# shahruk10/kaldi-tflite

Measured on AMD Instinct MI355X. Metric: x-vectors/sec (10 s @16 kHz), higher is better.
Workload: dtype f16mx

## Files before the change

### kaldi-tflite_amd/csrc/tdnn_mx.hip

```cpp
#include "tdnn_mx_common.h"

#define MXP_ROWS 256
__global__ __launch_bounds__(MXP_ROWS) void mx_planes_kernel(const float* __restrict__ src, int64_t T, int64_t ld, int D,
                                                             const int32_t* __restrict__ lens, char* __restrict__ xh,
                                                             char* __restrict__ xl4, char* __restrict__ x4, char* __restrict__ xs) {
    __shared__ float tile[MXP_ROWS * 33];
    const int b = blockIdx.z, c = blockIdx.y, nch = gridDim.y;
    const int64_t t0 = (int64_t)blockIdx.x * MXP_ROWS;
    const int64_t len = lens ? (int64_t)lens[b] : T;
    if (t0 >= len) return;
    const int rows = (int)(len - t0 < MXP_ROWS ? len - t0 : MXP_ROWS);
    const int tid = threadIdx.x;
    const float* base = src + ((int64_t)b * T + t0) * ld + c * 32;
    const bool vec = (ld & 3) == 0 && ((uintptr_t)src & 15) == 0 && c * 32 + 32 <= ld;
#pragma unroll
    for (int k = 0; k < 8; ++k) {
        const int q = k * MXP_ROWS + tid, r = q >> 3, e4 = (q & 7) * 4;
        if (r < rows) {
            float v[4];
            if (vec) {
                const f32x4 t = *reinterpret_cast<const f32x4*>(base + (int64_t)r * ld + e4);
                const int nd = D - (c * 32 + e4);
                v[0] = nd > 0 ? t.x : 0.0f; v[1] = nd > 1 ? t.y : 0.0f; v[2] = nd > 2 ? t.z : 0.0f; v[3] = nd > 3 ? t.w : 0.0f;
            } else {
#pragma unroll
                for (int e = 0; e < 4; ++e) v[e] = (c * 32 + e4 + e < D) ? base[(int64_t)r * ld + e4 + e] : 0.0f;
            }
#pragma unroll
            for (int e = 0; e < 4; ++e) tile[r * 33 + e4 + e] = __builtin_amdgcn_fmed3f(v[e], -65504.0f, 65504.0f);
        }
    }
    __syncthreads();
    const int64_t rec0 = ((int64_t)b * nch + c) * T + t0;
    u32x4 hp[4];
    if (tid < rows) {
        float v[32];
#pragma unroll
        for (int e = 0; e < 32; ++e) v[e] = tile[tid * 33 + e];
        u32x4 l4, h4;
        unsigned sw;
        mx_encode32(v, hp, l4, h4, sw);
        *reinterpret_cast<u32x4*>(xl4 + (rec0 + tid) * 16) = l4;
        *reinterpret_cast<u32x4*>(x4 + (rec0 + tid) * 16) = h4;
        *reinterpret_cast<unsigned*>(xs + (rec0 + tid) * 4) = sw;
    }
    __syncthreads();
    unsigned* himg = reinterpret_cast<unsigned*>(tile);
    if (tid < rows) {
#pragma unroll
        for (int k = 0; k < 4; ++k) *reinterpret_cast<u32x4*>(himg + tid * 20 + k * 4) = hp[k];
    }
    __syncthreads();
#pragma unroll
    for (int k = 0; k < 4; ++k) {
        const int q = k * MXP_ROWS + tid, r = q >> 2;
        if (r < rows)
            *reinterpret_cast<u32x4*>(xh + rec0 * 64 + (int64_t)q * 16) = *reinterpret_cast<const u32x4*>(himg + r * 20 + (q & 3) * 4);
    }
}

extern "C" int ktf_mx_planes(const float* src, int64_t B, int64_t T, int32_t D, int64_t ld_src, const int32_t* lens, void* xh,
                             void* xl4, void* x4, void* xs, void* stream) {
    KTF_REQUIRE(B >= 0 && T >= 0 && D > 0 && ld_src >= D, "ktf_mx_planes: bad size");
    if (B == 0 || T == 0) return KTF_OK;
    KTF_REQUIRE(src && xh && xl4 && x4 && xs, "ktf_mx_planes: null argument");
    const int nch = (D + 31) / 32;
    KTF_REQUIRE(B < 65536 && nch < 65536, "ktf_mx_planes: B and D / 32 must be below 65536");
    hipLaunchKernelGGL(mx_planes_kernel, dim3((unsigned)((T + MXP_ROWS - 1) / MXP_ROWS), (unsigned)nch, (unsigned)B), dim3(MXP_ROWS), 0,
                       (hipStream_t)stream, src, T, ld_src, (int)D, lens, (char*)xh, (char*)xl4, (char*)x4, (char*)xs);
    KTF_CHECK_LAUNCH("ktf_mx_planes");
    return KTF_OK;
}

template <int ACT, int OUT, bool PADK, bool FLAT = false>
__device__ __forceinline__ void mx_tile(const MxParams& p, const int id, int mtiles, int ntiles, int gtiles, double* __restrict__ stats,
                                        unsigned char* rsm) {
    static_assert(!FLAT || OUT != MX_OUT_F32, "flat row tiles: plane output or fused pooling");
#define MX_ARG_BATCH()                                                                                                                     \
    asm volatile("" ::"s"(p.xh), "s"(p.wh), "s"(p.T), "s"(p.nss), "s"(p.nk), "s"(p.nctx), "s"(p.nch_in), "s"(p.ctx_pk[0]), "s"(p.ctx_pk[1]), \
                 "s"(p.t_div_m), "s"(p.t_div_s), "s"(p.start), "s"(p.sub), "s"(p.cut))
    const int xcd = id & 7, slot = id >> 3;
    const int g = (slot / ntiles) * 8 + xcd;
    const int nt = slot - (slot / ntiles) * ntiles;
    if (g >= gtiles) return;
    const int b = FLAT ? 0 : g / mtiles, mt = FLAT ? g : g - b * mtiles;
    const int n0 = nt * 256, t0 = FLAT ? 0 : mt * 256;
    const int tid = threadIdx.x, lane = tid & 63;
    const int wave = __builtin_amdgcn_readfirstlane(tid >> 6);
    const int wm = wave >> 2, wn = wave & 3;
    const int R0 = mt * 256;
    int len, out_len;
    [[maybe_unused]] bool dense = false;
    if constexpr (FLAT) {
        const int total = p.row_starts[mtiles];
        MX_ARG_BATCH();
        if (R0 >= total) return;
        len = (int)p.T;
        out_len = total - R0 < 256 ? total - R0 : 256;
        dense = total == mtiles * len;
    } else {
        len = p.lens ? p.lens[b] : (int)p.T;
        MX_ARG_BATCH();
        out_len = len - p.cut - p.start <= 0 ? 0 : (len - p.cut - p.start + p.sub - 1) / p.sub;
        if (t0 >= out_len) return;
    }
    const int lenm1 = len - 1;
    const int64_t ub = FLAT ? 0 : (int64_t)b * p.nch_in * p.T;
    const int nkp = p.nss * 4;
    const __amdgpu_buffer_rsrc_t r_xh = mx_rsrc_pinned(p.xh + (ub - MX_KQ_BIAS) * 64);
    const __amdgpu_buffer_rsrc_t r_wh = mx_rsrc_pinned(p.wh + (int64_t)nt * nkp * MX_TILE);
    const __amdgpu_buffer_rsrc_t r_wq = mx_rsrc_pinned(p.wq + (int64_t)nt * p.nss * MX_WQ_BLOCK);

    unsigned a_cb[2];
    int a_row[2];
#pragma unroll
    for (int i = 0; i < 2; ++i) {
        const int q = i * 512 + tid;
        const int row = q >> 2;
        a_cb[i] = (unsigned)(((q & 3) ^ ((4 - ((row >> 2) & 3)) & 3)) * 16);
        a_row[i] = p.start + (t0 + row) * p.sub;
    }
    [[maybe_unused]] int a_lm1[2] = {lenm1, lenm1}, s_lm1 = lenm1;
    int s_row = p.start + (t0 + lane + 64 * (wave & 3)) * p.sub;
    [[maybe_unused]] unsigned a_ub[2] = {0u, 0u}, s_ub = 0u;
    [[maybe_unused]] auto flat_row = [&](int m) -> i32x4 {
        if (dense) {
            const int R = R0 + m;
            if (m >= out_len) return i32x4{-1, 0, 1, 0};
            const int bb = p.t_div_m ? (int)(__umulhi((unsigned)R, p.t_div_m) >> p.t_div_s) : R;
            return i32x4{R, R - bb * len, len, bb};
        }
        return reinterpret_cast<const i32x4*>(p.row_map)[R0 + m];
    };
    const unsigned long long cpk0 = p.ctx_pk[0], cpk1 = p.ctx_pk[1];
#define MX_CTX(ci_) ((int)(signed char)(((ci_) < 8 ? cpk0 : cpk1) >> (((ci_) & 7) * 8)))
    [[maybe_unused]] bool interior = false;
    if constexpr (FLAT) {
        i32x4 er[3];
        const int mr[3] = {tid >> 2, (512 + tid) >> 2, lane + 64 * (wave & 3)};
        if (dense) {
#pragma unroll
            for (int i = 0; i < 3; ++i) er[i] = flat_row(mr[i]);
        } else {
#pragma unroll
            for (int i = 0; i < 3; ++i) er[i] = reinterpret_cast<const i32x4*>(p.row_map)[R0 + mr[i]];
        }
#pragma unroll
        for (int i = 0; i < 2; ++i) {
            a_row[i] = er[i].y;
            a_lm1[i] = er[i].z - 1;
            a_ub[i] = er[i].x < 0 ? 0u : (unsigned)(er[i].x - er[i].y) * (unsigned)p.nch_in;
        }
        s_row = er[2].y;
        s_lm1 = er[2].z - 1;
        s_ub = er[2].x < 0 ? 0u : (unsigned)(er[2].x - er[2].y) * (unsigned)p.nch_in;
    }
    const unsigned vw = (unsigned)tid * 16u;
    const int wave_k0 = (int)(unsigned)(size_t)(lds_ptr_t*)(rsm + wave * 1024);
    [[maybe_unused]] const int wave_k = wave_k0;
#define MX_LDS_AT(off_, c_) ((lds_ptr_t*)(size_t)(unsigned)((off_) + (c_)))
    int kb[5], ko[5];
    kb[0] = MX_KQ_BIAS;
    ko[0] = MX_CTX(0);
#define MX_DMA_A_E(ks_, e_, n_)                                                                                        \
    {                                                                                                                  \
        int r_ = a_row[n_] + ko[e_];                                                                                   \
        const int hi_ = FLAT ? a_lm1[n_] : lenm1;                                                                      \
        r_ = r_ < 0 ? 0 : (r_ > hi_ ? hi_ : r_);                                                                       \
        const unsigned vo_ = ((FLAT ? a_ub[n_] : 0u) + (unsigned)r_) * 64u + a_cb[n_];                                 \
        __builtin_amdgcn_raw_ptr_buffer_load_lds(r_xh, MX_LDS_AT(wave_k, ((ks_) & 1) * MX_STAGE + (n_) * 8192), 16, vo_, kb[e_] << 6, 0, 0); \
    }
#define MX_DMA_A_I(ks_, e_, n_)                                                                                        \
    __builtin_amdgcn_raw_ptr_buffer_load_lds(r_xh, MX_LDS_AT(wave_k, ((ks_) & 1) * MX_STAGE + (n_) * 8192), 16, (n_) ? va1 : va0, \
                                             (kb[e_] + ko[e_]) << 6, 0, 0);
#define MX_DMA_A(ks_, e_, n_) { if constexpr (INTERIOR) MX_DMA_A_I(ks_, e_, n_) else MX_DMA_A_E(ks_, e_, n_) }
#define MX_DMA_W(ks_, n_)                                                                                              \
    __builtin_amdgcn_raw_ptr_buffer_load_lds(r_wh, MX_LDS_AT(wave_k, ((ks_) & 1) * MX_STAGE + MX_TILE + (n_) * 8192), 16, vw, \
                                             (ks_) * MX_TILE + (n_) * 8192, 0, 0);
    MX_DMA_W(0, 0) MX_DMA_W(0, 1) MX_DMA_A_E(0, 0, 0) MX_DMA_A_E(0, 0, 1)
    const __amdgpu_buffer_rsrc_t r_xl4 = mx_rsrc_pinned(p.xl4 + (ub - MX_KQ_BIAS) * 16);
    const __amdgpu_buffer_rsrc_t r_x4 = mx_rsrc_pinned(p.x4 + (ub - MX_KQ_BIAS) * 16);
    const __amdgpu_buffer_rsrc_t r_xs = mx_rsrc_pinned(p.xs + (ub - MX_KQ_BIAS) * 4);
    if constexpr (FLAT) {
        if (p.nctx == 1 && MX_CTX(0) == 0) {
            interior = true;
        } else if (out_len == 256) {
            const i32x4 e0 = flat_row(0), e1 = flat_row(255);
            interior = __builtin_amdgcn_readfirstlane(e0.w) == __builtin_amdgcn_readfirstlane(e1.w) &&
                       __builtin_amdgcn_readfirstlane(e0.y) + MX_CTX(0) >= 0 &&
                       __builtin_amdgcn_readfirstlane(e1.y) + MX_CTX(p.nctx - 1) <= __builtin_amdgcn_readfirstlane(e1.z) - 1;
        }
    }
    [[maybe_unused]] const unsigned va0 = (a_ub[0] + (unsigned)a_row[0]) * 64u + a_cb[0], va1 = (a_ub[1] + (unsigned)a_row[1]) * 64u + a_cb[1];
    [[maybe_unused]] const unsigned vs16 = (s_ub + (unsigned)s_row) * 16u, vs4 = (s_ub + (unsigned)s_row) * 4u;

    const int sa_k0 = (int)(unsigned)(size_t)(lds_ptr_t*)(rsm + (wave & 3) * 1024 + (wave >> 2) * 4096);
    const int sa_ks0 = (int)(unsigned)(size_t)(lds_ptr_t*)(rsm + (wave & 3) * 256 + (wave >> 2) * 1024);
    const bool wave_hi = wave >= 4;

    int* const tkb = reinterpret_cast<int*>(rsm + MX_KQ_OFF);
    int* const tko = tkb + (nkp + 4);

#define MX_DMA_SA(n_)                                                                                                  \
    {                                                                                                                  \
        constexpr int plane_ = ((n_) < 4 ? (n_) : 0) >> 1, h_ = (n_) < 4 ? ((n_) & 1) : (n_) - 4;                      \
        unsigned rec_ = 0u;                                                                                            \
        int so_;                                                                                                       \
        if constexpr (INTERIOR) {                                                                                      \
            so_ = sk_b[h_] + sk_o[h_];                                                                                 \
        } else {                                                                                                       \
            int r_ = s_row + sk_o[h_];                                                                                 \
            const int hi_ = FLAT ? s_lm1 : lenm1;                                                                      \
            r_ = r_ < 0 ? 0 : (r_ > hi_ ? hi_ : r_);                                                                   \
            rec_ = (FLAT ? s_ub : 0u) + (unsigned)r_;                                                                  \
            so_ = sk_b[h_];                                                                                            \
        }                                                                                                              \
        if ((n_) < 4) {                                                                                                \
            __builtin_amdgcn_raw_ptr_buffer_load_lds(plane_ ? r_x4 : r_xl4, MX_LDS_AT(sa_k, MX_SA_OFF + plane_ * 16384 + h_ * 8192), 16, \
                                                     INTERIOR ? vs16 : rec_ * 16u, so_ << 4, 0, 0);                    \
        } else {                                                                                                       \
            __builtin_amdgcn_raw_ptr_buffer_load_lds(r_xs, MX_LDS_AT(sa_ks, MX_SA_OFF + 32768 + h_ * 2048), 4, INTERIOR ? vs4 : rec_ * 4u, so_ << 2, 0, 0); \
        }                                                                                                              \
    }
#define MX_DMA_SW(ss_, n_)                                                                                             \
    __builtin_amdgcn_raw_ptr_buffer_load_lds(r_wq, MX_LDS_AT(wave_k, MX_SW_OFF + (n_) * 8192), 16, vw, (ss_) * MX_WQ_BLOCK + (n_) * 8192, 0, 0);

    f32x4 acc[8][4];
    const int r16 = lane & 15, q4 = lane >> 4;
    const int fr = (4 - ((r16 >> 2) & 3)) & 3;
    const int coff = ((q4 ^ fr) << 4);
    const int a_row_off = (wm * 128 + r16) * 64 + coff;
    const int b_row_off = (wn * 64 + r16) * 64 + coff;
    const int klim = PADK ? p.nk : nkp;

    auto kloop = [&](auto itag) {
        constexpr bool INTERIOR = decltype(itag)::value;
        {
            unsigned char* const prm_w = rsm + MX_PRM_OFF + (wave & 3) * 256;
            const unsigned vcol = (unsigned)(n0 + (wave & 3) * 64 + lane) * 4u;
            const float* const vec0 = wave_hi ? p.scale : p.bias;
            if (vec0) __builtin_amdgcn_raw_ptr_buffer_load_lds(mx_rsrc(vec0, p.units * 4), (lds_ptr_t*)(prm_w + (wave_hi ? 1024 : 0)), 4, vcol, 0, 0, 0);
            else reinterpret_cast<float*>(prm_w + (wave_hi ? 1024 : 0))[lane] = wave_hi ? 1.0f : 0.0f;
            if (!wave_hi) {
                if (p.shift) __builtin_amdgcn_raw_ptr_buffer_load_lds(mx_rsrc(p.shift, p.units * 4), (lds_ptr_t*)(prm_w + 2048), 4, vcol, 0, 0, 0);
                else reinterpret_cast<float*>(prm_w + 2048)[lane] = 0.0f;
            }
        }
        for (int k = tid; k < nkp + 4; k += 512) {
            const int kk = k + 1 < p.nk ? k + 1 : 0;
            const int ch = kk / p.nctx, ci = kk - ch * p.nctx;
            tkb[k] = ch * (int)p.T + MX_KQ_BIAS;
            tko[k] = MX_CTX(ci);
        }
        {
            int ch = 0, ci = 0;
#pragma unroll
            for (int e = 1; e <= 4; ++e) {
                if (++ci == p.nctx) { ci = 0; ++ch; }
                const bool real = e < p.nk;
                kb[e] = (real ? ch * (int)p.T : 0) + MX_KQ_BIAS;
                ko[e] = real ? MX_CTX(ci) : MX_CTX(0);
            }
        }
#pragma unroll
        for (int i = 0; i < 8; ++i)
#pragma unroll
            for (int j = 0; j < 4; ++j) acc[i][j] = f32x4{0.0f, 0.0f, 0.0f, 0.0f};
        for (int ss = 0; ss < p.nss; ++ss) {
            i32x4 tb_n, to_n;
            int sk_b[2], sk_o[2];
            int wave_k = wave_k0, sa_k = sa_k0, sa_ks = sa_ks0;
            asm volatile("" : "+s"(wave_k), "+s"(sa_k), "+s"(sa_ks));
#pragma unroll
            for (int j = 0; j < 4; ++j) {
                const int ks = 4 * ss + j;
                if (j == 1 || j == 2) asm volatile("s_waitcnt vmcnt(6)" ::: "memory");
                else if (j == 0) asm volatile("s_waitcnt vmcnt(0) lgkmcnt(0)" ::: "memory");
                else asm volatile("s_waitcnt vmcnt(0)" ::: "memory");
                __builtin_amdgcn_s_barrier();
                asm volatile("" ::: "memory");
                const bool live = PADK ? ks < p.nk : true;
#define MX_NEXT() ({ int k1_ = ks + 1; asm volatile("" : "+s"(k1_)); k1_ < klim; })
                const unsigned char* sa = rsm + (ks & 1) * MX_STAGE;
                const unsigned char* sw = sa + MX_TILE;
                hfrag8 bh[4];
                hfrag8 a_cur, a_nx1;
                if (live) {
#pragma unroll
                    for (int jj = 0; jj < 4; ++jj) bh[jj] = *reinterpret_cast<const hfrag8*>(sw + b_row_off + jj * 1024);
                    a_cur = *reinterpret_cast<const hfrag8*>(sa + a_row_off);
                    a_nx1 = *reinterpret_cast<const hfrag8*>(sa + a_row_off + 1024);
                }
                __builtin_amdgcn_sched_barrier(0);
                if (MX_NEXT()) { MX_DMA_A(ks + 1, j + 1, 0) MX_DMA_A(ks + 1, j + 1, 1) }
                __builtin_amdgcn_sched_barrier(0);
#pragma unroll
                for (int i = 0; i < 8; ++i) {
                    if (live) {
                        acc[i][0] = __builtin_amdgcn_mfma_f32_16x16x32_f16(a_cur, bh[0], acc[i][0], 0, 0, 0);
                        __builtin_amdgcn_sched_barrier(0);
                        hfrag8 a_nx2 = a_nx1;
                        if (i < 6) a_nx2 = *reinterpret_cast<const hfrag8*>(sa + a_row_off + (i + 2) * 1024);
#pragma unroll
                        for (int jj = 1; jj < 4; ++jj) acc[i][jj] = __builtin_amdgcn_mfma_f32_16x16x32_f16(a_cur, bh[jj], acc[i][jj], 0, 0, 0);
                        a_cur = a_nx1;
                        a_nx1 = a_nx2;
                    }
                    __builtin_amdgcn_sched_barrier(0);
                    if (i == 0) { if (MX_NEXT()) MX_DMA_W(ks + 1, 0) }
                    if (i == 1) { if (MX_NEXT()) MX_DMA_W(ks + 1, 1) }
                    if (j == 0) {
                        if (i == 1) {
                            sk_b[0] = wave_hi ? kb[1] : kb[0]; sk_o[0] = wave_hi ? ko[1] : ko[0];
                            sk_b[1] = wave_hi ? kb[3] : kb[2]; sk_o[1] = wave_hi ? ko[3] : ko[2];
                        }
                        if (i == 2) MX_DMA_SA(0)
                        if (i == 3) MX_DMA_SA(1)
                        if (i == 4) MX_DMA_SA(2)
                        if (i == 5) MX_DMA_SA(3)
                        if (i == 6) MX_DMA_SA(4)
                        if (i == 7) MX_DMA_SA(5)
                    }
                    if (j == 1) {
                        if (i == 2) MX_DMA_SW(ss, 0)
                        if (i == 3) MX_DMA_SW(ss, 1)
                        if (i == 4) MX_DMA_SW(ss, 2)
                        if (i == 5) MX_DMA_SW(ss, 3)
                        if (i == 6) MX_DMA_SW(ss, 4)
                        if (i == 7) MX_DMA_SW(ss, 5)
                    }
                    if (j == 2 && i == 3) {
                        tb_n = *reinterpret_cast<const i32x4*>(tkb + 4 * ss + 4);
                        to_n = *reinterpret_cast<const i32x4*>(tko + 4 * ss + 4);
                    }
                    __builtin_amdgcn_sched_barrier(0);
                }
#undef MX_NEXT
            }
            __builtin_amdgcn_sched_barrier(0);
            {
                int tl;
                asm volatile("v_mbcnt_lo_u32_b32 %0, -1, 0\n\tv_mbcnt_hi_u32_b32 %0, -1, %0" : "=v"(tl));
                const int sw_rec = ((tl & 63) >> 4) * 256 + wn * 64 + (tl & 15);
                const int sa_rec = ((tl & 63) >> 4) * 256 + wm * 128 + (tl & 15);
                unsigned o_a16 = MX_SA_OFF + sa_rec * 16, o_a4 = MX_SA_OFF + 32768 + sa_rec * 4;
                asm volatile("" : "+v"(o_a16), "+v"(o_a4));
                const unsigned char* const pa16 = rsm + o_a16;
                const unsigned char* const pa4 = rsm + o_a4;
                unsigned o_w16 = MX_SW_OFF + sw_rec * 16, o_w8 = MX_SW_OFF + 32768 + sw_rec * 8, o_w4 = MX_SW_OFF + 40960 + sw_rec * 4;
                asm volatile("" : "+v"(o_w16), "+v"(o_w8), "+v"(o_w4));
                const unsigned char* const pw16 = rsm + o_w16;
                const unsigned char* const pw8 = rsm + o_w8;
                const unsigned char* const pw4 = rsm + o_w4;
                u32x4 w4[4], wl6a[4];
                u32x2 wl6b[4];
                unsigned wsc[4];
#pragma unroll
                for (int jj = 0; jj < 4; ++jj) {
                    w4[jj] = *reinterpret_cast<const u32x4*>(pw16 + jj * 256);
                    wl6a[jj] = *reinterpret_cast<const u32x4*>(pw16 + 16384 + jj * 256);
                    wl6b[jj] = *reinterpret_cast<const u32x2*>(pw8 + jj * 128);
                    wsc[jj] = *reinterpret_cast<const unsigned*>(pw4 + jj * 64);
                }
                u32x4 l_n = *reinterpret_cast<const u32x4*>(pa16);
                u32x4 h_n = *reinterpret_cast<const u32x4*>(pa16 + 16384);
                unsigned s_n = *reinterpret_cast<const unsigned*>(pa4);
#pragma unroll
                for (int i = 0; i < 8; ++i) {
                    const u32x4 l = l_n, h = h_n;
                    const unsigned asc = s_n;
                    if (i < 7) {
                        l_n = *reinterpret_cast<const u32x4*>(pa16 + (i + 1) * 256);
                        h_n = *reinterpret_cast<const u32x4*>(pa16 + 16384 + (i + 1) * 256);
                        s_n = *reinterpret_cast<const unsigned*>(pa4 + (i + 1) * 64);
                    }
                    const i32x8 al = i32x8{(int)l.x, (int)l.y, (int)l.z, (int)l.w, 0, 0, 0, 0};
                    const i32x8 ah = i32x8{(int)h.x, (int)h.y, (int)h.z, (int)h.w, 0, 0, 0, 0};
#pragma unroll
                    for (int jj = 0; jj < 4; ++jj) {
                        const i32x8 bw = i32x8{(int)w4[jj].x, (int)w4[jj].y, (int)w4[jj].z, (int)w4[jj].w, 0, 0, 0, 0};
                        acc[i][jj] = __builtin_amdgcn_mfma_scale_f32_16x16x128_f8f6f4(al, bw, acc[i][jj], 4, 4, 0, asc, 0, wsc[jj]);
                    }
#pragma unroll
                    for (int jj = 0; jj < 4; ++jj) {
                        const i32x8 bw = i32x8{(int)wl6a[jj].x, (int)wl6a[jj].y, (int)wl6a[jj].z, (int)wl6a[jj].w, (int)wl6b[jj].x, (int)wl6b[jj].y, 0, 0};
                        acc[i][jj] = __builtin_amdgcn_mfma_scale_f32_16x16x128_f8f6f4(ah, bw, acc[i][jj], 4, 2, 1, asc, 1, wsc[jj]);
                    }
                    if (i == 3) {
                        kb[0] = kb[4];
                        ko[0] = ko[4];
#pragma unroll
                        for (int e = 0; e < 4; ++e) {
                            kb[e + 1] = __builtin_amdgcn_readfirstlane(tb_n[e]);
                            ko[e + 1] = __builtin_amdgcn_readfirstlane(to_n[e]);
                        }
                    }
                    __builtin_amdgcn_sched_barrier(0);
                }
            }
        }
    };
    if constexpr (FLAT) {
        if (interior) kloop(std::true_type{});
        else kloop(std::false_type{});
    } else {
        kloop(std::false_type{});
    }
#undef MX_DMA_A
#undef MX_DMA_A_E
#undef MX_DMA_A_I
#undef MX_DMA_W
#undef MX_DMA_SA
#undef MX_DMA_SW
#undef MX_ARG_BATCH
#undef MX_LDS_AT
#undef MX_CTX

#include "tdnn_mx_epilogue.inc"
}

template <int ACT, int OUT, bool PADK, bool FLAT = false>
__global__ __launch_bounds__(512) void tdnn_mx_kernel(MxParams p, int mtiles, int ntiles, int gtiles, double* __restrict__ stats) {
    extern __shared__ __attribute__((aligned(16))) unsigned char rsm[];
    mx_tile<ACT, OUT, PADK, FLAT>(p, blockIdx.x, mtiles, ntiles, gtiles, stats, rsm);
}

static int mx_launch(const void* xh, const void* xl4, const void* x4, const void* xs, int64_t B, int64_t T, const int32_t* lens,
                     const KtfTdnnDesc* d, const void* wh, const void* wq, const float* bias, const float* scale, const float* shift,
                     void* yh, void* yl4, void* y4, void* ys, float* yf, int64_t ldy, double* stats, void* stream, const char* who,
                     const int32_t* row_starts = nullptr, const int32_t* row_map = nullptr) {
    KTF_REQUIRE(d && wh && wq, "%s: null argument", who);
    KTF_REQUIRE(d->gemm == KTF_GEMM_F16MX, "%s: needs KTF_GEMM_F16MX", who);
    KTF_REQUIRE(B >= 0 && T >= 0 && B < 65536, "%s: bad size", who);
    KTF_REQUIRE(B == 0 || T == 0 || (xh && xl4 && x4 && xs), "%s: null argument", who);
    if (const int rc = tdnn_check_desc(d, scale, shift, who); rc != KTF_OK) return rc;
    KTF_REQUIRE(d->subsampling <= 64, "%s: subsampling %d outside [1,64]", who, d->subsampling);
    const bool plain = !d->valid && d->subsampling == 1;
    KTF_REQUIRE(plain || !stats, "%s: the fused pooling takes SAME padding without subsampling", who);
    KTF_REQUIRE(d->act == KTF_ACT_NONE || d->act == KTF_ACT_RELU, "%s: fuses ReLU or no activation", who);
    KTF_REQUIRE(T * (int64_t)d->din_pad * 2 < (1ll << 31) - (1ll << 20), "%s: T * din_pad too large", who);
    KTF_REQUIRE((((int64_t)d->din_pad / 32 * d->nctx + 3) / 4) * 4 <= MX_KQ_MAX_STEPS || (d->flags & KTF_TDNN_MX_LOADER), "%s: more than %d K-steps (din_pad / 32 * contexts)", who, MX_KQ_MAX_STEPS);
    if (B == 0 || T == 0 || ktf_tdnn_out_len(T, d) <= 0) return KTF_OK;
    const int outs = (yh ? 1 : 0) + (yf ? 1 : 0) + (stats ? 1 : 0);
    KTF_REQUIRE(outs == 1, "%s: exactly one of the plane / fp32 / pooled outputs", who);
    if (yh) KTF_REQUIRE(yl4 && y4 && ys, "%s: a plane output needs all four planes", who);
    if (yf) KTF_REQUIRE(ldy >= d->units, "%s: ldy < units", who);
    if (B == 0 || T == 0) return KTF_OK;
    MxParams p;
    memset(&p, 0, sizeof(p));
    p.xh = (const char*)xh; p.xl4 = (const char*)xl4; p.x4 = (const char*)x4; p.xs = (const char*)xs;
    p.lens = lens; p.wh = (const char*)wh; p.wq = (const char*)wq; p.bias = bias; p.scale = scale; p.shift = shift;
    p.yh = (char*)yh; p.yl4 = (char*)yl4; p.y4 = (char*)y4; p.ys = (char*)ys; p.yf = yf; p.ldy = ldy; p.T = T;
    p.units = d->units; p.nch_in = d->din_pad / 32; p.nctx = d->nctx; p.nk = p.nch_in * d->nctx; p.nss = (p.nk + 3) / 4;
    p.nch_out = (d->units + 31) / 32;
    p.sub = d->subsampling;
    p.start = (d->valid && d->ctx[0] < 0) ? -d->ctx[0] : 0;
    p.cut = (d->valid && d->ctx[d->nctx - 1] > 0) ? d->ctx[d->nctx - 1] : 0;
    p.Tout = ktf_tdnn_out_len(T, d);
    if (p.Tout <= 0) return KTF_OK;
    KTF_REQUIRE(plain || !(d->flags & KTF_TDNN_MX_LOADER), "%s: the loader-wave kernel takes SAME padding without subsampling", who);
    const bool loader = (d->flags & KTF_TDNN_MX_LOADER) != 0;
    p.stat_slots = (stats && (d->flags & KTF_TDNN_DET_STATS)) ? (int32_t)ktf_mx_stats_slots(T, d->flags) : 0;
    for (int i = 0; i < d->nctx; ++i) {
        KTF_REQUIRE(d->ctx[i] >= -128 && d->ctx[i] <= 127, "%s: context offsets outside [-128, 127]", who);
        p.ctx_pk[i >> 3] |= (unsigned long long)(unsigned char)(signed char)d->ctx[i] << ((i & 7) * 8);
    }
    hipStream_t st = (hipStream_t)stream;
    const int o = stats ? MX_OUT_STATS : (yf ? MX_OUT_F32 : MX_OUT_PLANES);
    if (loader) {
        const int rc = mxl_launch(p, B, d->act, o, stats, st);
        if (rc != KTF_OK) return rc;
        KTF_CHECK_LAUNCH(who);
        return KTF_OK;
    }
    if (row_starts) {
        KTF_REQUIRE(row_map && plain && o != MX_OUT_F32 && !loader, "%s: flat row tiles take the row table, SAME padding, no subsampling, a plane or pooled output", who);
        p.stat_slots = (stats && (d->flags & KTF_TDNN_DET_STATS)) ? (int32_t)ktf_flat_stats_slots(T) : 0;
        KTF_REQUIRE(B <= 4095 && B * T * (int64_t)p.nch_in * 64 < (1ll << 32) - (1ll << 20) && B * T < (1ll << 31) / (p.nch_out > 0 ? p.nch_out : 1),
                    "%s: flat row tiles need B <= 4095 and B * T * din_pad * 2 < 2^32", who);
        p.row_starts = row_starts; p.row_map = row_map;
        if (T > 1) {
            uint32_t l = 0;
            while ((1ull << l) < (uint64_t)T) ++l;
            p.t_div_m = (uint32_t)((1ull << (31 + l)) / (uint64_t)T + 1);
            p.t_div_s = l - 1;
        }
        const int ntiles = ktf_cdiv(d->units, 256);
        const int64_t ftiles = ktf_cdiv(B * T, 256);
        const int64_t fblocks = grouped_blocks(ftiles, ntiles);
        tdnn_pick<MX_OUT_STATS, MX_OUT_PLANES>(o, [&](auto O) {
            tdnn_pick<KTF_ACT_RELU, KTF_ACT_NONE>(d->act, [&](auto A) {
                tdnn_pick<true, false>((p.nk & 3) != 0, [&](auto PADK) {
                    tdnn_launch_kernel<tdnn_mx_kernel<A, O, PADK, true>>("tdnn_mx_kernel<flat>", dim3((unsigned)fblocks), dim3(512), MX_LDS_TOTAL(p.nss * 4),
                                                                         MX_LDS_TOTAL(MX_KQ_MAX_STEPS), st, p, (int)B, ntiles, (int)ftiles, stats);
                });
            });
        });
        KTF_CHECK_LAUNCH(who);
        return KTF_OK;
    }
    const int mtiles = ktf_cdiv(p.Tout, 256), ntiles = ktf_cdiv(d->units, 256);
    const int64_t gtiles = B * mtiles;
    const int64_t nblocks = grouped_blocks(gtiles, ntiles);
    tdnn_pick<KTF_ACT_RELU, KTF_ACT_NONE>(d->act, [&](auto A) {
        tdnn_pick<MX_OUT_STATS, MX_OUT_F32, MX_OUT_PLANES>(o, [&](auto O) {
            tdnn_pick<true, false>((p.nk & 3) != 0, [&](auto PADK) {
                tdnn_launch_kernel<tdnn_mx_kernel<A, O, PADK>>("tdnn_mx_kernel", dim3((unsigned)nblocks), dim3(512), MX_LDS_TOTAL(p.nss * 4),
                                                               MX_LDS_TOTAL(MX_KQ_MAX_STEPS), st, p, mtiles, ntiles, (int)gtiles, stats);
            });
        });
    });
    KTF_CHECK_LAUNCH(who);
    return KTF_OK;
}

extern "C" int ktf_tdnn_mx(const void* xh, const void* xl4, const void* x4, const void* xs, int64_t B, int64_t T, const int32_t* lens,
                           const KtfTdnnDesc* d, const void* wh, const void* wq, const float* bias, const float* scale,
                           const float* shift, void* yh, void* yl4, void* y4, void* ys, float* yf, int64_t ldy, void* stream) {
    return mx_launch(xh, xl4, x4, xs, B, T, lens, d, wh, wq, bias, scale, shift, yh, yl4, y4, ys, yf, ldy, nullptr, stream, "ktf_tdnn_mx");
}

extern "C" int ktf_tdnn_mx_flat(const void* xh, const void* xl4, const void* x4, const void* xs, int64_t B, int64_t T, const int32_t* row_starts,
                                const int32_t* row_map, const KtfTdnnDesc* d, const void* wh, const void* wq, const float* bias, const float* scale,
                                const float* shift, void* yh, void* yl4, void* y4, void* ys, void* stream) {
    KTF_REQUIRE(B == 0 || T == 0 || (row_starts && row_map && yh), "ktf_tdnn_mx_flat: null argument");
    return mx_launch(xh, xl4, x4, xs, B, T, nullptr, d, wh, wq, bias, scale, shift, yh, yl4, y4, ys, nullptr, 0, nullptr, stream, "ktf_tdnn_mx_flat",
                     row_starts, row_map);
}

extern "C" int ktf_tdnn_mx_flat_stats(const void* xh, const void* xl4, const void* x4, const void* xs, int64_t B, int64_t T, const int32_t* row_starts,
                                      const int32_t* row_map, const KtfTdnnDesc* d, const void* wh, const void* wq, const float* bias,
                                      const float* scale, const float* shift, double* sums, void* stream) {
    KTF_REQUIRE(sums && (B == 0 || T == 0 || (row_starts && row_map)), "ktf_tdnn_mx_flat_stats: null argument");
    return mx_launch(xh, xl4, x4, xs, B, T, nullptr, d, wh, wq, bias, scale, shift, nullptr, nullptr, nullptr, nullptr, nullptr, 0, sums, stream,
                     "ktf_tdnn_mx_flat_stats", row_starts, row_map);
}

extern "C" int ktf_tdnn_mx_stats(const void* xh, const void* xl4, const void* x4, const void* xs, int64_t B, int64_t T,
                                 const int32_t* lens, const KtfTdnnDesc* d, const void* wh, const void* wq, const float* bias,
                                 const float* scale, const float* shift, double* sums, void* stream) {
    KTF_REQUIRE(sums, "ktf_tdnn_mx_stats: null sums");
    return mx_launch(xh, xl4, x4, xs, B, T, lens, d, wh, wq, bias, scale, shift, nullptr, nullptr, nullptr, nullptr, nullptr, 0, sums, stream,
                     "ktf_tdnn_mx_stats");
}

extern "C" int32_t ktf_mx_slot_rows(int32_t flags) { return (flags & KTF_TDNN_MX_LOADER) ? 96 : 128; }
extern "C" int64_t ktf_mx_stats_slots(int64_t T, int32_t flags) {
    if (!(flags & KTF_TDNN_MX_LOADER)) return ktf_stats_slots(T);
    return T <= 0 ? 2 : 2 * ((T + 191) / 192);
}
```

### kaldi-tflite_amd/csrc/tdnn_mx_common.h

```cpp
#pragma once
#include "tdnn_common.h"
#include "flat_stats.h"
#include <type_traits>

typedef __attribute__((ext_vector_type(8))) int i32x8;
typedef __attribute__((ext_vector_type(8))) _Float16 hfrag8;
typedef __attribute__((ext_vector_type(2))) unsigned u32x2;

#define MX_TILE 16384
#define MX_STAGE (2 * MX_TILE)
#define MX_SA_OFF (2 * MX_STAGE)
#define MX_SA_BYTES (2 * 16384 + 4096)
#define MX_SW_OFF (MX_SA_OFF + MX_SA_BYTES)
#define MX_WQ_BLOCK 49152
#define MX_PRM_OFF (MX_SW_OFF + MX_WQ_BLOCK)
#define MX_LDS_BYTES (MX_PRM_OFF + 3 * 256 * 4)
#define MX_KQ_OFF MX_LDS_BYTES
#define MX_KQ_BIAS 128
#define MX_KQ_MAX_STEPS 1144
#define MX_LDS_TOTAL(nkp) (MX_LDS_BYTES + 8 * ((nkp) + 4))
static_assert(8 * 64 * 68 * 4 <= MX_PRM_OFF, "epilogue staging regions");
#define MX_EPW_PITCH 68

struct MxParams {
    const char* xh;
    const char* xl4;
    const char* x4;
    const char* xs;
    const int32_t* lens;
    const char* wh;
    const char* wq;
    const float* bias;
    const float* scale;
    const float* shift;
    char* yh;
    char* yl4;
    char* y4;
    char* ys;
    float* yf;
    int64_t ldy;
    int64_t T;
    int64_t Tout;
    int32_t units, nch_in, nctx, nk, nss, nch_out, stat_slots;
    int32_t sub, start, cut;
    unsigned long long ctx_pk[2];
    const int32_t* row_starts;
    const int32_t* row_map;
    uint32_t t_div_m, t_div_s;
};

__device__ __forceinline__ __amdgpu_buffer_rsrc_t mx_rsrc(const void* ptr, int bytes = -1) {
    return __builtin_amdgcn_make_buffer_rsrc(const_cast<void*>(ptr), 0, bytes, 0x00020000);
}
typedef int mx_rs4 __attribute__((ext_vector_type(4)));
__device__ __forceinline__ __amdgpu_buffer_rsrc_t mx_rsrc_pinned(const void* ptr, int bytes = -1) {
    const unsigned long long a = (unsigned long long)ptr;
    mx_rs4 w{(int)(unsigned)a, (int)((unsigned)(a >> 32) & 0xffffu), bytes, 0x00020000};
    asm volatile("" : "+s"(w));
    __amdgpu_buffer_rsrc_t r;
    __builtin_memcpy(&r, &w, 16);
    return r;
}

__device__ __forceinline__ unsigned mx_fp4_scale_byte(float m) {
    const unsigned bits = __float_as_uint(m);
    int byte = (int)(bits >> 23) - 2 + ((bits & 0x7fffffu) >= 0x600000u ? 1 : 0);
    return (unsigned)(byte < 1 ? 1 : byte);
}


__device__ __forceinline__ int mx_unit(int cb, int m) { return (cb >> 1) * 32 + (m >> 2) * 8 + (cb & 1) * 4 + (m & 3); }

__device__ __forceinline__ void mx_transpose4(unsigned& a, unsigned& b, unsigned& c, unsigned& d) {
    auto r = __builtin_amdgcn_permlane16_swap(a, b, false, false); a = r[0]; b = r[1];
    r = __builtin_amdgcn_permlane16_swap(c, d, false, false); c = r[0]; d = r[1];
    r = __builtin_amdgcn_permlane32_swap(a, c, false, false); a = r[0]; c = r[1];
    r = __builtin_amdgcn_permlane32_swap(b, d, false, false); b = r[0]; d = r[1];
}

template <int N>
__device__ __forceinline__ void mx_encode8(const float (&v)[N][8], u32x4 (&hp)[N], unsigned (&l4)[N], unsigned (&h4)[N], unsigned (&sw)[N]) {
    typedef __attribute__((ext_vector_type(2))) float f2;
    typedef __attribute__((ext_vector_type(2))) _Float16 h2;
    float lo[N][8];
    unsigned hw[N][4];
    float mv[N], ml[N];
#pragma unroll
    for (int n = 0; n < N; ++n) { mv[n] = 0.0f; ml[n] = 0.0f; }
#pragma unroll
    for (int k = 0; k < 4; ++k) {
#pragma unroll
        for (int n = 0; n < N; ++n) {
            const float a = v[n][2 * k], b = v[n][2 * k + 1];
            const h2 hh = __builtin_convertvector(f2{a, b}, h2);
            hw[n][k] = __builtin_bit_cast(unsigned, hh);
            asm("v_fma_mix_f32 %0, -%1, 1.0, %2 op_sel_hi:[1,0,0]" : "=v"(lo[n][2 * k]) : "v"(hw[n][k]), "v"(a));
            asm("v_fma_mix_f32 %0, -%1, 1.0, %2 op_sel:[1,0,0] op_sel_hi:[1,0,0]" : "=v"(lo[n][2 * k + 1]) : "v"(hw[n][k]), "v"(b));
            asm("v_max3_f32 %0, |%1|, |%2|, %3" : "=v"(mv[n]) : "v"(a), "v"(b), "v"(mv[n]));
            asm("v_max3_f32 %0, |%1|, |%2|, %3" : "=v"(ml[n]) : "v"(lo[n][2 * k]), "v"(lo[n][2 * k + 1]), "v"(ml[n]));
        }
    }
#pragma unroll
    for (int step = 0; step < 2; ++step) {
        unsigned o[N][2][2];
#pragma unroll
        for (int n = 0; n < N; ++n) {
            if (step == 0) {
                auto r = __builtin_amdgcn_permlane16_swap(__float_as_uint(mv[n]), __float_as_uint(mv[n]), false, false);
                o[n][0][0] = r[0]; o[n][0][1] = r[1];
                r = __builtin_amdgcn_permlane16_swap(__float_as_uint(ml[n]), __float_as_uint(ml[n]), false, false);
                o[n][1][0] = r[0]; o[n][1][1] = r[1];
            } else {
                auto r = __builtin_amdgcn_permlane32_swap(__float_as_uint(mv[n]), __float_as_uint(mv[n]), false, false);
                o[n][0][0] = r[0]; o[n][0][1] = r[1];
                r = __builtin_amdgcn_permlane32_swap(__float_as_uint(ml[n]), __float_as_uint(ml[n]), false, false);
                o[n][1][0] = r[0]; o[n][1][1] = r[1];
            }
        }
#pragma unroll
        for (int n = 0; n < N; ++n) {
            asm("v_max_f32 %0, %1, %2" : "=v"(mv[n]) : "v"(o[n][0][0]), "v"(o[n][0][1]));
            asm("v_max_f32 %0, %1, %2" : "=v"(ml[n]) : "v"(o[n][1][0]), "v"(o[n][1][1]));
        }
    }
    float sh[N], sl[N];
#pragma unroll
    for (int n = 0; n < N; ++n) {
        const float mh = (float)(_Float16)mv[n];
        const unsigned bh = mx_fp4_scale_byte(mh), bl = mx_fp4_scale_byte(ml[n]);
        sh[n] = __uint_as_float(bh << 23);
        sl[n] = __uint_as_float(bl << 23);
        sw[n] = bl | (bh << 8);
    }
    unsigned xb[N][4], yb[N][4];
#pragma unroll
    for (int k = 0; k < 4; ++k) {
#pragma unroll
        for (int n = 0; n < N; ++n) {
            xb[n][k] = 0;
            yb[n][k] = 0;
        }
    }
#define MX_ENC8_S(s_)                                                                                                   \
    _Pragma("unroll") for (int n = 0; n < N; ++n) {                                                                    \
        xb[n][s_] = __builtin_amdgcn_cvt_scalef32_pk_fp4_f32(xb[n][s_], lo[n][2 * s_], lo[n][2 * s_ + 1], sl[n], s_);  \
        yb[n][s_] = __builtin_amdgcn_cvt_scalef32_pk_fp4_f16(yb[n][s_], __builtin_bit_cast(h2, hw[n][s_]), sh[n], s_); \
    }
    MX_ENC8_S(0) MX_ENC8_S(1) MX_ENC8_S(2) MX_ENC8_S(3)
#undef MX_ENC8_S
#pragma unroll
    for (int n = 0; n < N; ++n) {
        l4[n] = (xb[n][0] | xb[n][1]) | (xb[n][2] | xb[n][3]);
        h4[n] = (yb[n][0] | yb[n][1]) | (yb[n][2] | yb[n][3]);
        hp[n] = u32x4{hw[n][0], hw[n][1], hw[n][2], hw[n][3]};
    }
}

#define MX_OUT_PLANES 0
#define MX_OUT_F32 1
#define MX_OUT_STATS 2

typedef __attribute__((ext_vector_type(2))) float mx_f2;
typedef __attribute__((ext_vector_type(2))) _Float16 mx_h2;
__device__ __forceinline__ void mx_encode32(const float (&v)[32], u32x4 (&hp)[4], u32x4& l4, u32x4& h4, unsigned& sw) {
    float lo[32];
    unsigned hw[16];
    float mv = 0.0f, ml = 0.0f;
#pragma unroll
    for (int k = 0; k < 16; ++k) {
        const float a = v[2 * k], b = v[2 * k + 1];
        const mx_h2 hh = __builtin_convertvector(mx_f2{a, b}, mx_h2);
        hw[k] = __builtin_bit_cast(unsigned, hh);
        asm("v_fma_mix_f32 %0, -%1, 1.0, %2 op_sel_hi:[1,0,0]" : "=v"(lo[2 * k]) : "v"(hw[k]), "v"(a));
        asm("v_fma_mix_f32 %0, -%1, 1.0, %2 op_sel:[1,0,0] op_sel_hi:[1,0,0]" : "=v"(lo[2 * k + 1]) : "v"(hw[k]), "v"(b));
        asm("v_max3_f32 %0, |%1|, |%2|, %3" : "=v"(mv) : "v"(a), "v"(b), "v"(mv));
        asm("v_max3_f32 %0, |%1|, |%2|, %3" : "=v"(ml) : "v"(lo[2 * k]), "v"(lo[2 * k + 1]), "v"(ml));
    }
    const float mh = (float)(_Float16)mv;
    const unsigned bh = mx_fp4_scale_byte(mh), bl = mx_fp4_scale_byte(ml);
    const float sh = __uint_as_float(bh << 23), sl = __uint_as_float(bl << 23);
    unsigned wl[4], wh_[4];
#pragma unroll
    for (int k = 0; k < 4; ++k) {
        unsigned x = 0, y = 0;
#define MX_ENC_S(s_)                                                                                                   \
        x = __builtin_amdgcn_cvt_scalef32_pk_fp4_f32(x, lo[8 * k + 2 * s_], lo[8 * k + 2 * s_ + 1], sl, s_);           \
        y = __builtin_amdgcn_cvt_scalef32_pk_fp4_f16(y, __builtin_bit_cast(mx_h2, hw[4 * k + s_]), sh, s_);
        MX_ENC_S(0) MX_ENC_S(1) MX_ENC_S(2) MX_ENC_S(3)
#undef MX_ENC_S
        wl[k] = x;
        wh_[k] = y;
        hp[k] = u32x4{hw[4 * k], hw[4 * k + 1], hw[4 * k + 2], hw[4 * k + 3]};
    }
    l4 = u32x4{wl[0], wl[1], wl[2], wl[3]};
    h4 = u32x4{wh_[0], wh_[1], wh_[2], wh_[3]};
    sw = bl | (bh << 8);
}

__device__ __forceinline__ float mx_act(float v, int act) { return act == KTF_ACT_RELU ? fmaxf(v, 0.0f) : v; }

__device__ __forceinline__ void mx_stats_out(double* __restrict__ stats, const MxParams& p, int b, int slot, int n, double s, double q) {
    if (p.stat_slots > 0) {
        double* dst = stats + (((int64_t)b * p.stat_slots + slot) * 2) * p.units + n;
        dst[0] = s;
        dst[p.units] = q;
    } else {
        double* dst = stats + ((int64_t)b * 2) * p.units + n;
        atomicAdd(dst, s);
        atomicAdd(dst + p.units, q);
    }
}

int mxl_launch(const MxParams& p, int64_t B, int act, int out_kind, double* stats, hipStream_t st);
```

Baseline: 112,300.

## Add contiguous-tile k-loop variant that fetches activation scales in one DMA

Adds a third k-loop specialization (CONTIG) for flat tiles whose 256 rows sit inside one utterance with all context offsets in range. In that case the activation scale DMAs 4 and 5 are merged into one per-wave load, issued alongside the last weight-scale load, and the vmcnt wait at j==1 is relaxed to match. Parameter and k-queue setup moves out of the per-variant lambda, and lane-derived values are recomputed with mbcnt inside each variant to reduce live registers. The change adds another template instantiation and relies on an exact count of outstanding loads for the new wait, which is a correctness risk.

Result: no change. 112,200 (median of 2 runs) (-0.1%).

```diff
diff --git a/kaldi-tflite_amd/csrc/tdnn_mx.hip b/kaldi-tflite_amd/csrc/tdnn_mx.hip
--- a/kaldi-tflite_amd/csrc/tdnn_mx.hip
+++ b/kaldi-tflite_amd/csrc/tdnn_mx.hip
@@ -134,16 +134,29 @@
     };
     const unsigned long long cpk0 = p.ctx_pk[0], cpk1 = p.ctx_pk[1];
 #define MX_CTX(ci_) ((int)(signed char)(((ci_) < 8 ? cpk0 : cpk1) >> (((ci_) & 7) * 8)))
-    [[maybe_unused]] bool interior = false;
+    constexpr bool USE_CONTIG = OUT != MX_OUT_STATS;
+    [[maybe_unused]] bool interior = false, contig = false;
+    [[maybe_unused]] unsigned c_rec = 0u;
+    [[maybe_unused]] int f_x0 = 0, f_y0 = 0, f_u0 = 0, f_y1 = 0, f_n1 = 1, f_u1 = 0;
     if constexpr (FLAT) {
         i32x4 er[3];
         const int mr[3] = {tid >> 2, (512 + tid) >> 2, lane + 64 * (wave & 3)};
+        const bool need_ends = USE_CONTIG || !(p.nctx == 1 && MX_CTX(0) == 0);
         if (dense) {
 #pragma unroll
             for (int i = 0; i < 3; ++i) er[i] = flat_row(mr[i]);
+            if (need_ends) {
+                const i32x4 e0 = flat_row(0), e1 = flat_row(255);
+                f_x0 = e0.x; f_y0 = e0.y; f_u0 = e0.w; f_y1 = e1.y; f_n1 = e1.z; f_u1 = e1.w;
+            }
         } else {
 #pragma unroll
             for (int i = 0; i < 3; ++i) er[i] = reinterpret_cast<const i32x4*>(p.row_map)[R0 + mr[i]];
+            if (need_ends) {
+                const i32x4 e0 = reinterpret_cast<const i32x4*>(p.row_map)[R0], e1 = reinterpret_cast<const i32x4*>(p.row_map)[R0 + 255];
+                f_x0 = __builtin_amdgcn_readfirstlane(e0.x); f_y0 = __builtin_amdgcn_readfirstlane(e0.y); f_u0 = __builtin_amdgcn_readfirstlane(e0.w);
+                f_y1 = __builtin_amdgcn_readfirstlane(e1.y); f_n1 = __builtin_amdgcn_readfirstlane(e1.z); f_u1 = __builtin_amdgcn_readfirstlane(e1.w);
+            }
         }
 #pragma unroll
         for (int i = 0; i < 2; ++i) {
@@ -182,14 +195,11 @@
     const __amdgpu_buffer_rsrc_t r_x4 = mx_rsrc_pinned(p.x4 + (ub - MX_KQ_BIAS) * 16);
     const __amdgpu_buffer_rsrc_t r_xs = mx_rsrc_pinned(p.xs + (ub - MX_KQ_BIAS) * 4);
     if constexpr (FLAT) {
-        if (p.nctx == 1 && MX_CTX(0) == 0) {
-            interior = true;
-        } else if (out_len == 256) {
-            const i32x4 e0 = flat_row(0), e1 = flat_row(255);
-            interior = __builtin_amdgcn_readfirstlane(e0.w) == __builtin_amdgcn_readfirstlane(e1.w) &&
-                       __builtin_amdgcn_readfirstlane(e0.y) + MX_CTX(0) >= 0 &&
-                       __builtin_amdgcn_readfirstlane(e1.y) + MX_CTX(p.nctx - 1) <= __builtin_amdgcn_readfirstlane(e1.z) - 1;
-        }
+        if (out_len == 256 && (USE_CONTIG || !(p.nctx == 1 && MX_CTX(0) == 0))) {
+            contig = f_u0 == f_u1 && f_y0 + MX_CTX(0) >= 0 && f_y1 + MX_CTX(p.nctx - 1) <= f_n1 - 1;
+            c_rec = (unsigned)(f_x0 - f_y0) * (unsigned)p.nch_in + (unsigned)f_y0;
+        }
+        interior = contig || (p.nctx == 1 && MX_CTX(0) == 0);
     }
     [[maybe_unused]] const unsigned va0 = (a_ub[0] + (unsigned)a_row[0]) * 64u + a_cb[0], va1 = (a_ub[1] + (unsigned)a_row[1]) * 64u + a_cb[1];
     [[maybe_unused]] const unsigned vs16 = (s_ub + (unsigned)s_row) * 16u, vs4 = (s_ub + (unsigned)s_row) * 4u;
@@ -225,43 +235,61 @@
 #define MX_DMA_SW(ss_, n_)                                                                                             \
     __builtin_amdgcn_raw_ptr_buffer_load_lds(r_wq, MX_LDS_AT(wave_k, MX_SW_OFF + (n_) * 8192), 16, vw, (ss_) * MX_WQ_BLOCK + (n_) * 8192, 0, 0);
 
+#define MX_DMA_S5(ss_)                                                                                                 \
+    {                                                                                                                  \
+        int w_ = wave;                        \
+        asm volatile("" : "+s"(w_));                                                                                   \
+        const bool hi_ = w_ >= 4;                                                                                      \
+        const int q0_ = kb[0] + ko[0], q1_ = kb[1] + ko[1], q2_ = kb[2] + ko[2], q3_ = kb[3] + ko[3];                  \
+        const int qa_ = (w_ & 1) ? q1_ : q0_, qb_ = (w_ & 1) ? q3_ : q2_;                                              \
+        const int kq_ = (w_ & 2) ? qb_ : qa_;                                                                          \
+        unsigned vl_;                            \
+        asm volatile("v_mbcnt_lo_u32_b32 %0, -1, 0\n\tv_mbcnt_hi_u32_b32 %0, -1, %0\n\tv_lshlrev_b32 %0, 4, %0" : "=v"(vl_)); \
+        int so_hi_ = (int)(c_rec + (unsigned)kq_) << 2, so_lo_ = (ss_) * MX_WQ_BLOCK + 5 * 8192 + w_ * 1024;              \
+        asm volatile("" : "+s"(so_hi_), "+s"(so_lo_));       \
+        __builtin_amdgcn_raw_ptr_buffer_load_lds(hi_ ? r_xs : r_wq, MX_LDS_AT(wave_k, hi_ ? MX_SA_OFF + 32768 - 4096 : MX_SW_OFF + 5 * 8192), \
+                                                 16, vl_, hi_ ? so_hi_ : so_lo_, 0, 0);                                \
+    }
+
     f32x4 acc[8][4];
-    const int r16 = lane & 15, q4 = lane >> 4;
-    const int fr = (4 - ((r16 >> 2) & 3)) & 3;
-    const int coff = ((q4 ^ fr) << 4);
-    const int a_row_off = (wm * 128 + r16) * 64 + coff;
-    const int b_row_off = (wn * 64 + r16) * 64 + coff;
     const int klim = PADK ? p.nk : nkp;
 
+    {
+        unsigned char* const prm_w = rsm + MX_PRM_OFF + (wave & 3) * 256;
+        const unsigned vcol = (unsigned)(n0 + (wave & 3) * 64 + lane) * 4u;
+        const float* const vec0 = wave_hi ? p.scale : p.bias;
+        if (vec0) __builtin_amdgcn_raw_ptr_buffer_load_lds(mx_rsrc(vec0, p.units * 4), (lds_ptr_t*)(prm_w + (wave_hi ? 1024 : 0)), 4, vcol, 0, 0, 0);
+        else reinterpret_cast<float*>(prm_w + (wave_hi ? 1024 : 0))[lane] = wave_hi ? 1.0f : 0.0f;
+        if (!wave_hi) {
+            if (p.shift) __builtin_amdgcn_raw_ptr_buffer_load_lds(mx_rsrc(p.shift, p.units * 4), (lds_ptr_t*)(prm_w + 2048), 4, vcol, 0, 0, 0);
+            else reinterpret_cast<float*>(prm_w + 2048)[lane] = 0.0f;
+        }
+    }
+    for (int k = tid; k < nkp + 4; k += 512) {
+        const int kk = k + 1 < p.nk ? k + 1 : 0;
+        const int ch = kk / p.nctx, ci = kk - ch * p.nctx;
+        tkb[k] = ch * (int)p.T + MX_KQ_BIAS;
+        tko[k] = MX_CTX(ci);
+    }
+    {
+        int ch = 0, ci = 0;
+#pragma unroll
+        for (int e = 1; e <= 4; ++e) {
+            if (++ci == p.nctx) { ci = 0; ++ch; }
+            const bool real = e < p.nk;
+            kb[e] = (real ? ch * (int)p.T : 0) + MX_KQ_BIAS;
+            ko[e] = real ? MX_CTX(ci) : MX_CTX(0);
+        }
+    }
     auto kloop = [&](auto itag) {
-        constexpr bool INTERIOR = decltype(itag)::value;
-        {
-            unsigned char* const prm_w = rsm + MX_PRM_OFF + (wave & 3) * 256;
-            const unsigned vcol = (unsigned)(n0 + (wave & 3) * 64 + lane) * 4u;
-            const float* const vec0 = wave_hi ? p.scale : p.bias;
-            if (vec0) __builtin_amdgcn_raw_ptr_buffer_load_lds(mx_rsrc(vec0, p.units * 4), (lds_ptr_t*)(prm_w + (wave_hi ? 1024 : 0)), 4, vcol, 0, 0, 0);
-            else reinterpret_cast<float*>(prm_w + (wave_hi ? 1024 : 0))[lane] = wave_hi ? 1.0f : 0.0f;
-            if (!wave_hi) {
-                if (p.shift) __builtin_amdgcn_raw_ptr_buffer_load_lds(mx_rsrc(p.shift, p.units * 4), (lds_ptr_t*)(prm_w + 2048), 4, vcol, 0, 0, 0);
-                else reinterpret_cast<float*>(prm_w + 2048)[lane] = 0.0f;
-            }
-        }
-        for (int k = tid; k < nkp + 4; k += 512) {
-            const int kk = k + 1 < p.nk ? k + 1 : 0;
-            const int ch = kk / p.nctx, ci = kk - ch * p.nctx;
-            tkb[k] = ch * (int)p.T + MX_KQ_BIAS;
-            tko[k] = MX_CTX(ci);
-        }
-        {
-            int ch = 0, ci = 0;
-#pragma unroll
-            for (int e = 1; e <= 4; ++e) {
-                if (++ci == p.nctx) { ci = 0; ++ch; }
-                const bool real = e < p.nk;
-                kb[e] = (real ? ch * (int)p.T : 0) + MX_KQ_BIAS;
-                ko[e] = real ? MX_CTX(ci) : MX_CTX(0);
-            }
-        }
+        constexpr bool INTERIOR = decltype(itag)::value != MX_K_EDGE, CONTIG = decltype(itag)::value == MX_K_CONTIG;
+        int kl;
+        asm volatile("v_mbcnt_lo_u32_b32 %0, -1, 0\n\tv_mbcnt_hi_u32_b32 %0, -1, %0" : "=v"(kl));
+        const int r16 = kl & 15, q4 = (kl >> 4) & 3;
+        const int fr = (4 - ((r16 >> 2) & 3)) & 3;
+        const int coff = ((q4 ^ fr) << 4);
+        const int a_row_off = (wm * 128 + r16) * 64 + coff;
+        const int b_row_off = (wn * 64 + r16) * 64 + coff;
 #pragma unroll
         for (int i = 0; i < 8; ++i)
 #pragma unroll
@@ -274,7 +302,8 @@
 #pragma unroll
             for (int j = 0; j < 4; ++j) {
                 const int ks = 4 * ss + j;
-                if (j == 1 || j == 2) asm volatile("s_waitcnt vmcnt(6)" ::: "memory");
+                if (j == 1 && CONTIG) asm volatile("s_waitcnt vmcnt(4)" ::: "memory");
+                else if (j == 1 || j == 2) asm volatile("s_waitcnt vmcnt(6)" ::: "memory");
                 else if (j == 0) asm volatile("s_waitcnt vmcnt(0) lgkmcnt(0)" ::: "memory");
                 else asm volatile("s_waitcnt vmcnt(0)" ::: "memory");
                 __builtin_amdgcn_s_barrier();
@@ -318,8 +347,10 @@
                         if (i == 3) MX_DMA_SA(1)
                         if (i == 4) MX_DMA_SA(2)
                         if (i == 5) MX_DMA_SA(3)
-                        if (i == 6) MX_DMA_SA(4)
-                        if (i == 7) MX_DMA_SA(5)
+                        if constexpr (!CONTIG) {
+                            if (i == 6) MX_DMA_SA(4)
+                            if (i == 7) MX_DMA_SA(5)
+                        }
                     }
                     if (j == 1) {
                         if (i == 2) MX_DMA_SW(ss, 0)
@@ -327,7 +358,7 @@
                         if (i == 4) MX_DMA_SW(ss, 2)
                         if (i == 5) MX_DMA_SW(ss, 3)
                         if (i == 6) MX_DMA_SW(ss, 4)
-                        if (i == 7) MX_DMA_SW(ss, 5)
+                        if (i == 7) { if constexpr (CONTIG) MX_DMA_S5(ss) else MX_DMA_SW(ss, 5) }
                     }
                     if (j == 2 && i == 3) {
                         tb_n = *reinterpret_cast<const i32x4*>(tkb + 4 * ss + 4);
@@ -401,10 +432,16 @@
         }
     };
     if constexpr (FLAT) {
-        if (interior) kloop(std::true_type{});
-        else kloop(std::false_type{});
+        if constexpr (USE_CONTIG) {
+            if (!interior) kloop(std::integral_constant<int, MX_K_EDGE>{});
+            else if (contig) kloop(std::integral_constant<int, MX_K_CONTIG>{});
+            else kloop(std::integral_constant<int, MX_K_INTERIOR>{});
+        } else {
+            if (interior) kloop(std::integral_constant<int, MX_K_INTERIOR>{});
+            else kloop(std::integral_constant<int, MX_K_EDGE>{});
+        }
     } else {
-        kloop(std::false_type{});
+        kloop(std::integral_constant<int, MX_K_EDGE>{});
     }
 #undef MX_DMA_A
 #undef MX_DMA_A_E
@@ -412,11 +449,17 @@
 #undef MX_DMA_W
 #undef MX_DMA_SA
 #undef MX_DMA_SW
+#undef MX_DMA_S5
 #undef MX_ARG_BATCH
 #undef MX_LDS_AT
 #undef MX_CTX
 
+    {
+        int lane_e;
+        asm volatile("v_mbcnt_lo_u32_b32 %0, -1, 0\n\tv_mbcnt_hi_u32_b32 %0, -1, %0" : "=v"(lane_e));
+        [[maybe_unused]] const int lane = lane_e, q4 = lane_e >> 4;
 #include "tdnn_mx_epilogue.inc"
+    }
 }
 
 template <int ACT, int OUT, bool PADK, bool FLAT = false>
diff --git a/kaldi-tflite_amd/csrc/tdnn_mx_common.h b/kaldi-tflite_amd/csrc/tdnn_mx_common.h
--- a/kaldi-tflite_amd/csrc/tdnn_mx_common.h
+++ b/kaldi-tflite_amd/csrc/tdnn_mx_common.h
@@ -19,6 +19,9 @@
 #define MX_KQ_BIAS 128
 #define MX_KQ_MAX_STEPS 1144
 #define MX_LDS_TOTAL(nkp) (MX_LDS_BYTES + 8 * ((nkp) + 4))
+#define MX_K_EDGE 0
+#define MX_K_INTERIOR 1
+#define MX_K_CONTIG 2
 static_assert(8 * 64 * 68 * 4 <= MX_PRM_OFF, "epilogue staging regions");
 #define MX_EPW_PITCH 68
 
```
